# LasseWolter/laughter-detection-icsi

Measured on AMD Instinct MI355X. Metric: 1 s@16 kHz segments/sec (featurize+ResNet fwd/bwd), higher is better.
Workload: dtype f32 (64->64 and 32->32 convolutions: f16x2 split operands with per-tile power-of-two scales, f32 accumulate; error vs float64 within 1.5x of the exact-f32 kernels'); 1 GPU; BASELINE configs[2]: end-to-end featurize (HIP fbank 44 mel) + ResNetBigger resnet_base fwd/bwd + clip + Adam, random labels, dropout 0.5; global_batch=512, parallelism=dp1, overlap_wgrad=False, overlap_wgrad_small=True, bf16x3_convs=True, f16x2_convs=True, relu_bits=True, virtual_a1=True

## Files before the change

include/lad_hip.h:

```cpp
#ifndef LAD_HIP_H
#define LAD_HIP_H

#include <stdint.h>

#ifdef __cplusplus
extern "C" {
#endif

#define LAD_VERSION 100

enum lad_status {
    LAD_OK = 0,
    LAD_ERR_INVALID = -1,
    LAD_ERR_HIP = -2,
    LAD_ERR_NOMEM = -3,
    LAD_NOT_COVERED = 1
};

int lad_version(void);
const char *lad_last_error(void);

enum lad_pad_mode {
    LAD_PAD_KALDI_MIRROR = 0,
    LAD_PAD_CENTER_REFLECT = 1,
// ... 36 lines not shown
                         int32_t band, int32_t row_bytes, void *stream);


int64_t lad_act_rows(int64_t batch, int32_t H, int32_t W);

int64_t lad_conv_packed_weight_floats(int32_t cout, int32_t cin, int32_t taps, int32_t mode);
int lad_conv_pack_weights(const float *w, int32_t cout, int32_t cin, int32_t taps, int32_t mode, float *wt,
                          void *stream);
int lad_conv_pack_weights_multi(const void *descs, int32_t n_desc, void *stream);
int64_t lad_conv_num_tiles(int64_t batch, int32_t H, int32_t W);
int lad_conv_fwd(const float *in, const float *wt, const float *bias, const float *addend, float *out,
                 float *stat_partials, int64_t batch, int32_t H, int32_t W, int32_t cin, int32_t cout, int32_t taps,
                 void *stream);
int lad_conv_s2_fwd(const float *in, const float *wt, const float *bias, float *out, float *stat_partials,
                    int64_t batch, int32_t H, int32_t W, int32_t cin, int32_t cout, int32_t taps, void *stream);
int lad_bn_fold(const float *gamma, const float *beta, const float *running_mean, const float *running_var,
                const float *conv_bias, int32_t channels, float *scale, float *shift, void *stream);
int lad_conv_fwd_eval(const float *in, const float *wt, const float *scale, const float *shift, const float *addend,
                      float *out, int64_t batch, int32_t H, int32_t W, int32_t cin, int32_t cout, int32_t taps,
                      int32_t relu, void *stream);
int lad_conv_s2_fwd_eval(const float *in, const float *wt, const float *scale, const float *shift, float *out,
                         int64_t batch, int32_t H, int32_t W, int32_t cin, int32_t cout, int32_t taps, int32_t relu,
                         void *stream);
int lad_upsample2(const float *src, float *up, int64_t batch, int32_t H, int32_t W, int32_t channels, void *stream);
int lad_conv_s2_dgrad(const float *dout, const float *wt, float *dx, int64_t batch, int32_t H, int32_t W, int32_t cin,
                      int32_t cout, int32_t taps, int32_t accumulate, void *stream);
int64_t lad_conv_s2_wgrad_workspace_floats(int32_t cin, int32_t cout, int32_t taps);
int lad_conv_s2_wgrad(const float *in, const float *dout, float *workspace, float *dw, float *dbias, int64_t batch, int32_t H,
                      int32_t W, int32_t cin, int32_t cout, int32_t taps, void *stream);
int64_t lad_conv_s2_wgrad_fused_workspace_floats(int32_t cin, int32_t cout);
int lad_conv_s2_wgrad_fused(const float *in, const float *dout, const float *dout_sc, float *workspace, float *dw,
                            float *dbias, float *dw_sc, int64_t batch, int32_t H, int32_t W, int32_t cin, int32_t cout,
                            void *stream);
int lad_conv_s2_fwd_fused(const float *in, const float *wt, const float *bias, const float *wt_sc, float *out,
                          float *stat_partials, float *out_sc, float *stat_partials_sc, int64_t batch, int32_t H, int32_t W,
                          int32_t cin, int32_t cout, void *stream);
int lad_conv_s2_dgrad_fused(const float *dout, const float *wt, const float *dout_sc, const float *wt_sc, float *dx,
                            int64_t batch, int32_t H, int32_t W, int32_t cin, int32_t cout, void *stream);
int64_t lad_conv_s2b3_packed_weight_bytes(void);
int lad_conv_s2b3_pack_weights(const float *w, const float *w_sc, void *wt, void *stream);
int lad_conv_s2b3_fwd(const float *in, const void *wt, const float *bias, float *out, float *stat_partials, float *out_sc,
                      float *stat_partials_sc, int64_t batch, int32_t H, int32_t W, void *stream);
int64_t lad_conv_s2b3_dgrad_packed_weight_bytes(void);
int lad_conv_s2b3_dgrad_pack_weights(const float *w, const float *w_sc, void *wt, void *stream);
int lad_conv_s2b3_pack_weights_pair(const float *w, const float *w_sc, void *wt_fwd, void *wt_dgrad, void *stream);
int64_t lad_conv_s2b3_dgrad_partials(int64_t batch, int32_t H, int32_t W);
int lad_conv_s2b3_dgrad(const float *dout, const float *dout_sc, const void *wt, float *dx, float *stat_partials, const float *bn_x,
                        const uint64_t *bn_bits, const float *bn_coef, int64_t batch, int32_t H, int32_t W, void *stream);
int64_t lad_conv_s2_dgrad_partials(int64_t batch, int32_t H, int32_t W);
int lad_conv_s2_dgrad_fused_bnstat(const float *dout, const float *wt, const float *dout_sc, const float *wt_sc, float *dx,
                                   float *stat_partials, const float *bn_x, const uint64_t *bn_bits, const float *bn_coef,
                                   int64_t batch, int32_t H, int32_t W, int32_t cin, int32_t cout, void *stream);
int64_t lad_conv_wgrad_workspace_floats(int32_t cin, int32_t cout, int32_t taps);
int lad_conv_wgrad(const float *in, const float *dout, float *workspace, float *dw, float *dbias, int64_t batch,
                   int32_t H, int32_t W, int32_t cin, int32_t cout, int32_t taps, void *stream);

int64_t lad_conv_b3_packed_weight_bytes(void);
int lad_conv_b3_pack_weights(const float *w, int32_t mode, void *wt, void *stream);
int lad_conv_b3_fwd_f32(const float *in, const void *wt, const float *bias, const float *addend, float *out,
                        float *partials, int64_t batch, int32_t H, int32_t W, void *stream);
int lad_conv_b3_fwd_f32_gated(const float *in, const void *wt, const float *bias, const float *addend,
                              const uint64_t *addend_bits, float *out, float *partials, int64_t batch, int32_t H,
                              int32_t W, void *stream);
int lad_conv_b3_dgrad_bnstat(const float *in, const void *wt, const float *addend, const uint64_t *addend_bits,
                             float *out, float *stat_partials, const float *bn_x, const uint64_t *bn_bits,
                             const float *bn_coef, int64_t batch, int32_t H, int32_t W, void *stream);
// ... 188 lines not shown
```

laughter-detection-icsi_amd/_hip.py:

```python
import ctypes
import os

import torch

_HERE = os.path.dirname(os.path.abspath(__file__))
LIB_PATH = os.environ.get("LAD_HIP_LIB") or os.path.join(_HERE, "liblad_hip.so")

c_void_p = ctypes.c_void_p
c_int = ctypes.c_int
c_i64 = ctypes.c_int64
c_float = ctypes.c_float
c_double = ctypes.c_double
c_i32 = ctypes.c_int32
c_float_p = ctypes.POINTER(ctypes.c_float)


class LadHipError(RuntimeError):
    pass


class FbankCfg(ctypes.Structure):
    _fields_ = [("n_fft", ctypes.c_int32), ("frame_len", ctypes.c_int32), ("hop", ctypes.c_int32),
                ("n_mels", ctypes.c_int32), ("n_mfcc", ctypes.c_int32), ("pad_mode", ctypes.c_int32),
                ("log_mode", ctypes.c_int32), ("remove_dc", ctypes.c_int32), ("preemph", ctypes.c_float),
# ... 32 lines not shown
    "lad_conv_wgrad_h2": (c_int, [c_void_p] * 6 + [c_i64, c_i32, c_i32, c_i32, c_void_p]),
    "lad_conv_h2": (c_int, [c_void_p] * 11 + [c_i64, c_i32, c_i32, c_i32, c_void_p]),
    "lad_conv_wgrad_h2_bnbwd": (c_int, [c_void_p] * 11 + [c_i64, c_i32, c_i32, c_i32, c_void_p]),
    "lad_conv_wgrad_b3c_workspace_floats": (c_i64, [c_i32]),
    "lad_conv_wgrad_b3c": (c_int, [c_void_p] * 6 + [c_i64, c_i32, c_i32, c_i32, c_void_p]),
    "lad_conv_b3_fwd_f32_gated": (c_int, [c_void_p] * 7 + [c_i64, c_i32, c_i32, c_void_p]),
    "lad_conv_b3_fwd_f32_bnrelu": (c_int, [c_void_p] * 6 + [c_i64, c_i32, c_i32, c_void_p]),
    "lad_conv_wgrad_b3_bnrelu": (c_int, [c_void_p] * 6 + [c_i64, c_i32, c_i32, c_void_p]),
    "lad_wgrad_defer_begin": (c_int, []),
    "lad_wgrad_defer_flush": (c_int, [c_void_p]),
    "lad_conv_b3_dgrad_bnstat": (c_int, [c_void_p] * 9 + [c_i64, c_i32, c_i32, c_void_p]),
    "lad_conv_wgrad_b3": (c_int, [c_void_p] * 5 + [c_i64, c_i32, c_i32, c_void_p]),
    "lad_conv_s2_fwd": (c_int, [c_void_p] * 5 + [c_i64, c_i32, c_i32, c_i32, c_i32, c_i32, c_void_p]),
    "lad_bn_fold": (c_int, [c_void_p] * 5 + [c_i32, c_void_p, c_void_p, c_void_p]),
    "lad_conv_fwd_eval": (c_int, [c_void_p] * 6 + [c_i64, c_i32, c_i32, c_i32, c_i32, c_i32, c_i32, c_void_p]),
    "lad_conv_s2_fwd_eval": (c_int, [c_void_p] * 5 + [c_i64, c_i32, c_i32, c_i32, c_i32, c_i32, c_i32, c_void_p]),
    "lad_upsample2": (c_int, [c_void_p, c_void_p, c_i64, c_i32, c_i32, c_i32, c_void_p]),
    "lad_conv_s2_dgrad": (c_int, [c_void_p] * 3 + [c_i64, c_i32, c_i32, c_i32, c_i32, c_i32, c_i32, c_void_p]),
    "lad_conv_s2_wgrad_workspace_floats": (c_i64, [c_i32, c_i32, c_i32]),
    "lad_conv_s2_fwd_fused": (c_int, [c_void_p] * 8 + [c_i64, c_i32, c_i32, c_i32, c_i32, c_void_p]),
    "lad_conv_s2_dgrad_partials": (c_i64, [c_i64, c_i32, c_i32]),
    "lad_conv_s2b3_packed_weight_bytes": (c_i64, []),
    "lad_conv_s2b3_pack_weights": (c_int, [c_void_p, c_void_p, c_void_p, c_void_p]),
    "lad_conv_s2b3_fwd": (c_int, [c_void_p] * 7 + [c_i64, c_i32, c_i32, c_void_p]),
    "lad_conv_s2b3_dgrad_packed_weight_bytes": (c_i64, []),
    "lad_conv_s2b3_dgrad_pack_weights": (c_int, [c_void_p, c_void_p, c_void_p, c_void_p]),
    "lad_conv_s2b3_pack_weights_pair": (c_int, [c_void_p] * 5),
    "lad_conv_s2b3_dgrad_partials": (c_i64, [c_i64, c_i32, c_i32]),
    "lad_conv_s2b3_dgrad": (c_int, [c_void_p] * 8 + [c_i64, c_i32, c_i32, c_void_p]),
    "lad_conv_s2_dgrad_fused_bnstat": (c_int, [c_void_p] * 9 + [c_i64, c_i32, c_i32, c_i32, c_i32, c_void_p]),
    "lad_conv_s2_dgrad_fused": (c_int, [c_void_p] * 5 + [c_i64, c_i32, c_i32, c_i32, c_i32, c_void_p]),
    "lad_conv_s2_wgrad_fused_workspace_floats": (c_i64, [c_i32, c_i32]),
    "lad_conv_s2_wgrad_fused": (c_int, [c_void_p] * 7 + [c_i64, c_i32, c_i32, c_i32, c_i32, c_void_p]),
    "lad_conv_s2_wgrad": (c_int, [c_void_p] * 5 + [c_i64, c_i32, c_i32, c_i32, c_i32, c_i32, c_void_p]),
    "lad_conv_wgrad_workspace_floats": (c_i64, [c_i32, c_i32, c_i32]),
    "lad_conv_wgrad": (c_int, [c_void_p] * 5 + [c_i64, c_i32, c_i32, c_i32, c_i32, c_i32, c_void_p]),
    "lad_stem_fwd": (c_int, [c_void_p] * 4 + [c_i64, c_i32, c_i32, c_i32, c_void_p]),
    "lad_stem_fwd_eval": (c_int, [c_void_p] * 5 + [c_i64, c_i32, c_i32, c_i32, c_i64, c_i64, c_void_p]),
    "lad_stem_wgrad_workspace_floats": (c_i64, []),
    "lad_stem_wgrad": (c_int, [c_void_p] * 4 + [c_i64, c_i32, c_i32, c_i32, c_void_p]),
    "lad_stem_wgrad_bn": (c_int, [c_void_p] * 8 + [c_i64, c_i32, c_i32, c_i32, c_void_p]),
    "lad_stem_bn_bwd_groups": (c_i64, [c_i64, c_i32, c_i32]),
    "lad_stem_bn_bwd_sums": (c_int, [c_void_p] * 5 + [c_i64, c_i32, c_i32, c_i32, c_void_p]),
    "lad_bn_finalize": (c_int, [c_void_p, c_i64, c_i32, c_i64, c_void_p, c_void_p, c_void_p, c_void_p, c_float,
                                c_void_p, c_void_p]),
    "lad_stem_moments_workspace_doubles": (c_i64, []),
    "lad_stem_moments_doubles": (c_i64, []),
    "lad_stem_bn_stats": (c_int, [c_void_p] * 6 + [c_float] + [c_void_p] * 3 + [c_i64, c_i32, c_i32, c_i32, c_void_p]),
    "lad_stem_bwd_onepass_workspace_floats": (c_i64, []),
    "lad_stem_bwd_onepass": (c_int, [c_void_p] * 10 + [c_i64, c_i32, c_i32, c_i32, c_void_p]),
    "lad_bn_finalize_pair": (c_int, [c_void_p, c_void_p, c_i64, c_i32, c_i64] + [c_void_p] * 10 + [c_float, c_void_p]),
    "lad_bn_act": (c_int, [c_void_p] * 5 + [c_i64, c_i32, c_i32, c_i32, c_i32, c_void_p]),
    "lad_bn_bwd_workspace_floats": (c_i64, [c_i32]),
    "lad_bn_act_bits": (c_int, [c_void_p] * 6 + [c_i64, c_i32, c_i32, c_i32, c_void_p]),
    "lad_bn_bwd_bits": (c_int, [c_void_p] * 11 + [c_i64, c_i64, c_i32, c_i32, c_i32, c_void_p]),
    "lad_bn_bwd": (c_int, [c_void_p] * 17 + [c_i64, c_i64, c_i32, c_i32, c_i32, c_i32, c_i32, c_void_p]),
    "lad_conv_fwd_bnstat": (c_int, [c_void_p] * 8 + [c_i64, c_i32, c_i32, c_i32, c_i32, c_i32, c_void_p]),
    "lad_pool_fwd": (c_int, [c_void_p, c_void_p, c_i64, c_i32, c_i32, c_i32, c_void_p]),
    "lad_pool_bwd": (c_int, [c_void_p, c_void_p, c_i64, c_i32, c_i32, c_i32, c_void_p]),
    "lad_head_workspace_floats": (c_i64, [c_i64, c_i32]),
    "lad_head_fwd_train": (c_int, [c_void_p, c_void_p, c_i64, c_i32, c_void_p, c_void_p, c_void_p, c_float,
                                   c_void_p, c_void_p, c_void_p, c_void_p, c_void_p]),
    "lad_head_fwd_train_rng": (c_int, [c_void_p, c_void_p, c_i64, c_i32, c_void_p, c_void_p, c_float, ctypes.c_uint64, c_void_p, c_void_p, c_i32,
                                       c_void_p, c_float, c_void_p, c_void_p, c_void_p, c_void_p, c_void_p]),
    "lad_head_fwd_eval": (c_int, [c_void_p, c_void_p, c_i64, c_i32, c_void_p, c_void_p]),
    "lad_bce_metrics": (c_int, [c_void_p, c_void_p, c_i64, c_void_p, c_void_p]),
# ... 93 lines not shown
```

laughter-detection-icsi_amd/engine.py:

```python
import ctypes
import math
import struct
from typing import FrozenSet, NamedTuple, Optional, Tuple

import torch

import _hip

_VP = ctypes.c_void_p


PREDICT_CHUNK = {"fp16": 8192, "fp32": 2048}
BASE_WIDTHS = (64, 32, 16, 16)
STREAM_SUPER_MAX = 1 << 20


class _LazyLevels(dict):

    def __init__(self, make):
        super().__init__()
        self._make = make

    def __missing__(self, key):
        value = self[key] = self._make(key)
# ... 27 lines not shown
        self.wt_d = image(lib.lad_conv_packed_weight_floats(cout, cin, taps, 1), torch.float32)
        self.wt_h = image(lib.lad_f16_packed_weight_halfs(cout, cin, taps), torch.float16)
        if _b3_shape(cin, cout, taps, stride) and base_widths:
            self.wt3_f, self.wt3_d = (image(lib.lad_conv_b3c_packed_weight_bytes(cin), torch.uint8) for _ in range(2))
            self.wt2_f, self.wt2_d = (image(lib.lad_conv_h2_packed_weight_bytes(cin), torch.uint8) for _ in range(2))
        if _s2b3_shape(cin, cout, taps, stride) and base_widths:
            self.wt3_s2f = image(lib.lad_conv_s2b3_packed_weight_bytes(), torch.uint8)
            self.wt3_s2d = image(lib.lad_conv_s2b3_dgrad_packed_weight_bytes(), torch.uint8)


class _BnParams:

    def __init__(self, name, c, views, bufs, dev, conv_bias=None):
        self.name, self.c, self.conv_bias = name, c, conv_bias
        self.g, self.gg = views[name + ".weight"]
        self.b, self.gb = views[name + ".bias"]
        self.rm, self.rv = bufs[name + ".running_mean"], bufs[name + ".running_var"]
        if not (self.rm.is_cuda and self.rm.is_contiguous() and self.rm.dtype == torch.float32):
            raise _hip.LadHipError(f"{name}: running statistics must be contiguous float32 GPU tensors")
        self.fold = (torch.zeros(c, device=dev), torch.zeros(c, device=dev))


class _ConvSpec:

    def __init__(self, name, cin, cout, taps, stride, h_in, w_in, base_widths=True):
        self.name, self.cin, self.cout, self.taps, self.stride = name, cin, cout, taps, stride
        self.h_in, self.w_in = h_in, w_in
        self.h_out = (h_in + stride - 1) // stride
        self.w_out = (w_in + stride - 1) // stride
        self.b3 = _b3_shape(cin, cout, taps, stride) and w_in <= 46 and base_widths
        self.b3_full = self.b3 and cin == 64
        self.b3_wgrad = self.b3 and (cin == 64 or w_in <= 30)
        self.s2b3 = _s2b3_shape(cin, cout, taps, stride) and (w_in + 1) // 2 <= 45 and base_widths
        self.par = None

    def rows(self, B):
        return B * (self.h_in + 1) * (self.w_in + 1) + self.w_in + 2


class _BlockSpec:

    def __init__(self, name):
        self.name = name
        self.conv1 = self.bn1 = self.conv2 = self.bn2 = self.sc_conv = self.sc_bn = None


def block_geometry(stem_cout, filter_sizes, H, W, base_widths):
    blocks = []
    cin, h, w = stem_cout, H, W
    for bi, cout in enumerate(filter_sizes, start=1):
        for j in range(2):
            name = f"block{bi}.{j}"
            stride = 2 if (j == 0 and bi > 1) else 1
            b = _BlockSpec(name)
            b.conv1 = _ConvSpec(name + ".conv1", cin, cout, 9, stride, h, w, base_widths)
            h, w = b.conv1.h_out, b.conv1.w_out
            b.conv2 = _ConvSpec(name + ".conv2", cout, cout, 9, 1, h, w, base_widths)
            if stride != 1 or cin != cout:
                b.sc_conv = _ConvSpec(name + ".shortcut.0", cin, cout, 1, stride, b.conv1.h_in, b.conv1.w_in, base_widths)
            blocks.append(b)
            cin = cout
    return blocks


class _ConvChoice(NamedTuple):
    arith: str
    wgrad: str
    wgrad_bn: bool
    label_fwd: str
    label_dgrad: str


class _BlockChoice(NamedTuple):
    entry: str
    a1_virtual: bool
    bits: bool
    dgrad2_bn: Optional[str]
    dgrad1_bn: Optional[str]
    sc_wgrad_fused: bool
    conv1: _ConvChoice
    conv2: _ConvChoice
    sc: Optional[_ConvChoice]


class _TrainSchedule(NamedTuple):
    blocks: Tuple[_BlockChoice, ...]
    stem_onepass: bool
    images: FrozenSet[Tuple[str, str]]
    opts: Tuple[Tuple[str, object], ...]


_ROW_LIMIT = (1 << 31) - (1 << 20)


def train_schedule(blocks, B, opts, stem_onepass):
    o = dict(opts)

    def arith(cs):
        fits = cs.rows(B) < _ROW_LIMIT if cs.cin == 64 else cs.rows(B) * cs.cin * 4 < _ROW_LIMIT
        if not (o["bf16x3"] and cs.b3 and (cs.cin == 64 or o["bf16x3_32"]) and fits):
            return "f32"
        return "h2" if o["f16x2"] and (cs.cin == 64 or o["f16x2_32"]) else "b3"

    def conv(cs, dgrad_f32=False, label_fwd=None):
        a = arith(cs)
        wg = "f32" if a == "f32" or not cs.b3_wgrad else "h2" if a == "h2" and cs.cin == 64 else "b3c"
        f32_label = f"conv_s{cs.stride}<{cs.cin},{cs.cout},{cs.taps}>"
        return _ConvChoice(a, wg, bool(o["fuse_bn_bwd_wgrad"]) and wg == "h2",
                           label_fwd or (f32_label if a == "f32" else f"conv_{a}<{cs.cin},{cs.cout},{cs.taps}>"),
                           f"conv_s1<{cs.cout},{cs.cin},{cs.taps}>" if a == "f32" or dgrad_f32 else f"conv_{a}<{cs.cout},{cs.cin},{cs.taps}>")

    out = []
    for bi, b in enumerate(blocks):
        c1, c2, sc = b.conv1, b.conv2, b.sc_conv
        a1, a2 = arith(c1), arith(c2)
        below_bits = bi > 0 and out[bi - 1].bits
        entry = "plain"
        if c1.stride != 1 and o["fuse_s2_shortcut"]:
            entry = "s2b3" if o["bf16x3"] and o["s2_b3"] and c1.s2b3 and c1.rows(B) < _ROW_LIMIT else "s2_fused"
        bits = bool(o["relu_bits"]) and sc is None and c1.b3_full and a1 != "f32" and not o["fuse_bn_bwd"]
        dgrad2_bn = "f32" if o["fuse_bn_bwd"] else "split" if o["fuse_bn_bwd_b3"] and a2 != "f32" else None
        if c1.stride != 1:
            fused = entry == "s2b3" or (entry == "s2_fused" and c1.cin == 64 and c1.cout == 32)
            dgrad1_bn = "split" if fused and o["fuse_bn_bwd_b3"] and below_bits else None
        elif bits:
            dgrad1_bn = "split" if o["fuse_bn_bwd_b3"] and below_bits else None
        else:
            dgrad1_bn = "f32" if o["fuse_bn_bwd"] and bi > 0 and blocks[bi - 1].sc_conv is None else None
        s2_label = f"conv_{'s2b3' if entry == 's2b3' else 's2'}<{c1.cin},{c1.cout},9>" if c1.stride != 1 else None
        out.append(_BlockChoice(entry, bool(o["virtual_a1"]) and a2 != "f32" and c2.b3_wgrad, bits, dgrad2_bn, dgrad1_bn,
                                c1.stride != 1 and bool(o["fuse_s2_shortcut_wgrad"]),
                                conv(c1, dgrad1_bn == "f32", s2_label), conv(c2, dgrad2_bn == "f32"), conv(sc) if sc is not None else None))
    images = {(ch.arith if ch.arith == "h2" else "b3c", cs.name) for b, blk in zip(blocks, out)
              for cs, ch in ((b.conv1, blk.conv1), (b.conv2, blk.conv2)) if ch.arith != "f32"}
    images |= {("s2b3", b.conv1.name) for b, blk in zip(blocks, out) if blk.entry == "s2b3"}
    return _TrainSchedule(tuple(out), bool(stem_onepass), frozenset(images), tuple(o.items()))


def conv_s1_entry(arith, cin, in_coef=False, gated=False, bn=None):
    if arith == "h2" and bn != "y":
        return "lad_conv_h2"
    if arith == "b3" and in_coef and not gated and bn is None:
        return "lad_conv_b3c_fwd_f32_bnrelu"
    if arith == "b3" and gated and not in_coef and cin == 64 and bn in (None, "bits"):
        return "lad_conv_b3_dgrad_bnstat" if bn else "lad_conv_b3_fwd_f32_gated"
    if arith == "b3" and not in_coef and not gated and bn in (None, "x"):
        return "lad_conv_b3c_dgrad_bnstat" if bn else "lad_conv_b3c_fwd_f32"
    if arith == "f32" and not in_coef and not gated and bn != "bits":
        return "lad_conv_fwd_bnstat" if bn else "lad_conv_fwd"
    raise _hip.LadHipError(f"no stride-1 convolution kernel for arithmetic {arith!r} at {cin} channels with in_coef={in_coef}, "
                           f"gated={gated}, bn={bn!r}")


def conv_wgrad_entry(kind, in_coef=False, bn=False):
    if kind == "h2":
        return "lad_conv_wgrad_h2_bnbwd" if bn else "lad_conv_wgrad_h2"
    if kind == "b3c" and not bn:
        return "lad_conv_wgrad_b3c"
    if kind == "f32" and not bn and not in_coef:
        return "lad_conv_wgrad"
    raise _hip.LadHipError(f"no weight-gradient kernel for {kind!r} with in_coef={in_coef}, bn={bn}")


def _s2_shortcut_rides(b, opts):
    return bool(opts["f16_s2_shortcut_fused"]) and b.conv1.cin != 32


def _block_fits_lds(b, B, opts, hw=None):
    c = b.conv1
# ... 135 lines not shown
        self.i0, self.S, self.B_max = i0, S, B_max
        self.base, self.frames_avail = base, frames_avail
        self.cat = self.cat2 = self.stem = None


class ResNetEngine:
    KERNEL_OPTIONS =("bf16x3", "bf16x3_32", "f16x2", "f16x2_32", "relu_bits", "virtual_a1", "fuse_bn_bwd", "fuse_bn_bwd_b3", "fuse_bn_bwd_wgrad", "fuse_s2_shortcut",
                      "fuse_s2_shortcut_wgrad", "s2_b3")
    INFER_OPTIONS = ("stream_direct", "stream_level2", "stream_super", "strip_block_fused", "small_block_fused", "tail_fused", "strip2_resident",
                     "strip_stem_shared", "f16_s2_shortcut_fused")

    def __init__(self, model):
        self.model = model
        self.device = None
        self._flat_p = self._flat_g = None
        self._plans = {}
        self._step_count = 0
        self._lib = None
        self._grad_dirty = False
        self._train_forwards = 0
        self._weights_version = 0
        self.fuse_bn_bwd = False
        self.overlap_wgrad = False
        self.overlap_wgrad_small = "auto"
        self.stem_onepass = True
        self.bf16x3 = True
        self.fuse_bn_bwd_b3 = True
        self.fuse_bn_bwd_wgrad = True
        self.f16x2 = True
        self.f16x2_32 = True
        self.bf16x3_32 = True
        self.virtual_a1 = True
        self.s2_b3 = True
        self.stream_direct = True
        self.stream_level2 = True
        self.strip_block_fused = True
        self.small_block_fused = True
        self.stream_super = True
        self.tail_fused = True
        self.strip2_resident = True
        self.strip_stem_shared = True
        self._sup_cache = {}
        self._sup_plans = {}
        self._layouts = {}
        self.f16_s2_shortcut_fused = True
        self.fuse_s2_shortcut = True
        self.fuse_s2_shortcut_wgrad = True
        self.defer_wgrad_sums = True
        self._defer_on = False
        self._schedules = {}
        self.relu_bits = True
        self._side = None
        self._side_readers = {}
        self._side_pending = False
        self.debug_capture = None
        self.kernel_events = None
        self.base_widths = list(model.filter_sizes) == list(BASE_WIDTHS)
        if not self.base_widths:
            for k in self.KERNEL_OPTIONS:
                setattr(self, k, False)

    def lib(self):
        if self._lib is None:
            self._lib = _hip.lib()
        return self._lib

    def _named_params(self):
        return list(self.model.named_parameters())

    def ensure_flat(self):
        params = self._named_params()
        dev = params[0][1].device
        if dev.type != "cuda":
            raise _hip.LadHipError("ResNetBigger runs on the MI355X only: call model.set_device('cuda') first "
                                   "(the HIP path has no CPU fallback)")
        ok = self._flat_p is not None and self._flat_p.device == dev
        if ok:
            base = self._flat_p.data_ptr()
            for (name, p), off in zip(params, self._offsets):
                if p.data_ptr() != base + 4 * off or p.dtype != torch.float32:
                    ok = False
                    break
        if ok:
            return
        offs, total = [], 0
        for _, p in params:
            offs.append(total)
            total += _align4(p.numel())
        flat_p = torch.zeros(total, device=dev, dtype=torch.float32)
        flat_g = torch.zeros(total, device=dev, dtype=torch.float32)
        with torch.no_grad():
            for (name, p), off in zip(params, offs):
# ... 237 lines not shown
            _hip.check(lib.lad_conv_h2_pack_weights_multi(_hip.ptr(htab[0]), htab[1], 0, st), "lad_conv_h2_pack_weights_multi")
        self._packed = (ver, need_dgrad or have[1], want | have[2]) if fresh else (ver, need_dgrad, want)

    def _eval_prepare(self, half):
        if not half:
            self._pack_weights(need_dgrad=False)
        tag = self._state_tag()
        lib, st = self.lib(), self._st()
        if self._folded != tag:
            for bn in (self.stem_bn, *self._bns.values()):
                _hip.check(lib.lad_bn_fold(_hip.ptr(bn.g), _hip.ptr(bn.b), _hip.ptr(bn.rm), _hip.ptr(bn.rv), _hip.ptr(bn.conv_bias),
                                           bn.c, _hip.ptr(bn.fold[0]), _hip.ptr(bn.fold[1]), st), "lad_bn_fold " + bn.name)
            self._folded = tag
        if half and self._f16_packed != tag:
            for par in self._convs.values():
                _hip.check(lib.lad_f16_pack_weights(_hip.ptr(par.w), par.cout, par.cin, par.taps, _hip.ptr(par.wt_h), st),
                           "lad_f16_pack_weights " + par.name)
            self._f16_packed = tag

    def _mark(self, label):
        if self.kernel_events is None or label not in self.kernel_events:
            return None
        ev = torch.cuda.Event(enable_timing=True)
        ev.record(torch.cuda.current_stream(self.device))
        return ev

    def _mark_end(self, label, start):
        if start is not None:
            ev = torch.cuda.Event(enable_timing=True)
            ev.record(torch.cuda.current_stream(self.device))
            self.kernel_events[label].append((start, ev))

    def _schedule(self, B, H, W):
        key = (B, H, W, self.stem_onepass) + tuple(getattr(self, k) for k in self.KERNEL_OPTIONS)
        sched = self._schedules.get(key)
        if sched is None:
            sched = self._schedules[key] = train_schedule(self._blocks_for(H, W)[0], B, {k: getattr(self, k) for k in self.KERNEL_OPTIONS},
                                                          self.stem_onepass)
        return sched

    def _conv_s1(self, cs, arith, direction, x, out, B, label=None, *, in_coef=None, bias=None, addend=None, abits=None, partials=None, bn=None):
        bx, bmask, bcoef = bn if bn is not None else (None, None, None)
        fn = conv_s1_entry(arith, cs.cin, in_coef is not None, abits is not None,
                           None if bn is None else "x" if bmask is None else "bits" if bmask.dtype == torch.int64 else "y")
        P, fwd, h, w = _hip.ptr, direction == "fwd", cs.h_in, cs.w_in
        wt = P(getattr(cs.par, {"h2": "wt2_", "b3": "wt3_", "f32": "wt_"}[arith] + ("f" if fwd else "d")))
        cio = (cs.cin, cs.cout) if fwd else (cs.cout, cs.cin)
        if fn == "lad_conv_h2":
            args = (P(x), P(in_coef), wt, P(bias), P(addend), P(abits), P(out), P(partials), P(bx), P(bmask), P(bcoef), B, h, w, cs.cin)
        elif fn == "lad_conv_b3c_fwd_f32":
            args = (P(x), wt, P(bias), P(addend), P(out), P(partials), B, h, w, cs.cin)
        elif fn == "lad_conv_b3c_fwd_f32_bnrelu":
            args = (P(x), P(in_coef), wt, P(bias), P(out), P(partials), B, h, w, cs.cin)
        elif fn == "lad_conv_b3c_dgrad_bnstat":
            args = (P(x), wt, P(addend), P(out), P(partials), P(bx), P(bcoef), B, h, w, cs.cin)
        elif fn == "lad_conv_b3_fwd_f32_gated":
            args = (P(x), wt, P(bias), P(addend), P(abits), P(out), P(partials), B, h, w)
        elif fn == "lad_conv_b3_dgrad_bnstat":
            args = (P(x), wt, P(addend), P(abits), P(out), P(partials), P(bx), P(bmask), P(bcoef), B, h, w)
        elif fn == "lad_conv_fwd":
            args = (P(x), wt, P(bias), P(addend), P(out), P(partials), B, h, w, *cio, cs.taps)
        else:
            args = (P(x), wt, P(addend), P(out), P(partials), P(bx), P(bmask), P(bcoef), B, h, w, *cio, cs.taps)
        t0 = self._mark(label)
        _hip.check(getattr(self.lib(), fn)(*args, self._st()), f"{fn}({direction}) {cs.name}")
        self._mark_end(label, t0)

    def _conv_fwd(self, cs, ch, x, out, partials, B, in_coef=None):
        if cs.stride == 1:
            self._conv_s1(cs, ch.arith, "fwd", x, out, B, ch.label_fwd, in_coef=in_coef, bias=cs.par.b, partials=partials)
            return
# ... 670 lines not shown
                self._bn_bwd(p, b.bn2, dy, a["y"], a["c2"], a["coef2"], dc2, B, ho, wo, 1, mode=2, aux=aux,
                             sbn=b.sc_bn, xs=a["cs"], scoef=a["coefs"])
            xin, xcoef = (a["c1"], a["coef1"]) if ch.a1_virtual else (a["a1"], None)
            self._conv_wgrad(p, c2s, ch.conv2.wgrad, xin, dc2, B, in_coef=xcoef, bn=(dy, a["c2"], bits, a["coef2"]) if fuse2 else None)
            stat = (a["c1"], None, a["coef1"]) if ch.dgrad2_bn else None
            self._conv_s1(c2s, "f32" if ch.dgrad2_bn == "f32" else ch.conv2.arith, "dgrad", dc2, da1, B, ch.conv2.label_dgrad,
                          bn=stat, partials=p["partials"] if stat else None)
            self._bn_bwd(p, b.bn1, da1, None, a["c1"], a["coef1"], None if fuse1 else dc1, B, ho, wo, 2, mode=0, pre=stat is not None)
            if c1s.stride == 1:
                self._conv_wgrad(p, c1s, ch.conv1.wgrad, a["x"], dc1, B, bn=(da1, a["c1"], None, a["coef1"]) if fuse1 else None)
            if self.debug_capture is not None:
                self.debug_capture[b.name] = {"dy": dy.clone(), "dc2": dc2.clone(), "aux": aux.clone() if bits is None else None, "da1": da1.clone(),
                                              "dc1": dc1.clone()}
            if c1s.stride == 1:
                dx = dy
                if b.sc_conv is not None:
                    self._conv_wgrad(p, b.sc_conv, ch.sc.wgrad, a["x"], aux, B)
                    self._conv_s1(b.sc_conv, ch.sc.arith, "dgrad", aux, da1, B)
                    aux = da1
                stat = (lower["c2"], lower["ybits" if ch.dgrad1_bn == "split" else "y"], lower["coef2"]) if ch.dgrad1_bn else None
                self._conv_s1(c1s, "f32" if ch.dgrad1_bn == "f32" else ch.conv1.arith, "dgrad", dc1, dx, B, ch.conv1.label_dgrad,
                              addend=dy if ch.bits else aux, abits=bits, bn=stat, partials=p["partials"] if stat else None)
                pre2, pre2_tiles = stat is not None, 0
            else:
                dx = p["g"][(hi, wi)][0]
                sc = b.sc_conv

                def s2_wgrad(cs, dout, xin=a["x"]):
                    self._on_side(lambda sst: _hip.check(lib.lad_conv_s2_wgrad(
                        _hip.ptr(xin), _hip.ptr(dout), _hip.ptr(self._wg_ws(p, cs)), _hip.ptr(cs.par.gw), _hip.ptr(cs.par.gb), B, hi, wi, cs.cin, cs.cout,
                        cs.taps, sst), "lad_conv_s2_wgrad " + cs.name), dout, small=cs.cin <= 32)

                if ch.sc_wgrad_fused:
                    self._on_side(lambda sst, c1s=c1s, sc=sc, dc1=dc1, aux=aux, xin=a["x"]: _hip.check(lib.lad_conv_s2_wgrad_fused(
                        _hip.ptr(xin), _hip.ptr(dc1), _hip.ptr(aux), _hip.ptr(self._wg_ws(p, c1s)), _hip.ptr(c1s.par.gw), _hip.ptr(c1s.par.gb),
                        _hip.ptr(sc.par.gw), B, hi, wi, c1s.cin, c1s.cout, sst), "lad_conv_s2_wgrad_fused " + c1s.name), dc1, small=c1s.cin <= 32)
                    if dc1.data_ptr() in self._side_readers:
                        self._side_readers[aux.data_ptr()] = self._side_readers[dc1.data_ptr()]
                else:
                    s2_wgrad(c1s, dc1)
                stat = (lower["c2"], lower["ybits"], lower["coef2"]) if ch.dgrad1_bn else (None, None, None)
                n_part = 0
                if ch.entry == "s2b3":
                    n_part = int(lib.lad_conv_s2b3_dgrad_partials(B, hi, wi))
                    assert not ch.dgrad1_bn or n_part * 2 * 64 <= p["partials"].numel()
                    _hip.check(lib.lad_conv_s2b3_dgrad(_hip.ptr(dc1), _hip.ptr(aux), _hip.ptr(c1s.par.wt3_s2d), _hip.ptr(dx),
                                                       _hip.ptr(p["partials"]) if ch.dgrad1_bn else None, _hip.ptr(stat[0]), _hip.ptr(stat[1]),
                                                       _hip.ptr(stat[2]), B, hi, wi, st), "lad_conv_s2b3_dgrad " + c1s.name)
                elif ch.entry == "s2_fused" and ch.dgrad1_bn:
                    n_part = int(lib.lad_conv_s2_dgrad_partials(B, hi, wi))
                    assert n_part * 2 * 64 <= p["partials"].numel()
                    _hip.check(lib.lad_conv_s2_dgrad_fused_bnstat(_hip.ptr(dc1), _hip.ptr(c1s.par.wt_d), _hip.ptr(aux), _hip.ptr(sc.par.wt_d), _hip.ptr(dx),
                                                                  _hip.ptr(p["partials"]), _hip.ptr(stat[0]), _hip.ptr(stat[1]),
                                                                  _hip.ptr(stat[2]), B, hi, wi, c1s.cin, c1s.cout, st),
                               "lad_conv_s2_dgrad_fused_bnstat " + c1s.name)
                elif ch.entry == "s2_fused":
                    _hip.check(lib.lad_conv_s2_dgrad_fused(_hip.ptr(dc1), _hip.ptr(c1s.par.wt_d), _hip.ptr(aux), _hip.ptr(sc.par.wt_d), _hip.ptr(dx),
                                                           B, hi, wi, c1s.cin, c1s.cout, st), "lad_conv_s2_dgrad_fused " + c1s.name)
                else:
                    _hip.check(lib.lad_conv_s2_dgrad(_hip.ptr(dc1), _hip.ptr(c1s.par.wt_d), _hip.ptr(dx), B, hi, wi, c1s.cin, c1s.cout, 9, 0,
                                                     st), "lad_conv_s2_dgrad " + c1s.name)
                pre2, pre2_tiles = ch.dgrad1_bn is not None, n_part
                if not ch.sc_wgrad_fused:
                    s2_wgrad(sc, aux)
                if ch.entry == "plain":
                    _hip.check(lib.lad_conv_s2_dgrad(_hip.ptr(aux), _hip.ptr(sc.par.wt_d), _hip.ptr(dx), B, hi, wi, sc.cin, sc.cout, 1, 1, st),
                               "lad_conv_s2_dgrad " + sc.name)
            dy = dx
        if sched.stem_onepass:
# ... 134 lines not shown
```

Measured before the change: 47960 segments/s.

## Add f16x2 split-precision MFMA kernel for fused stride-2 64->32 weight gradient

Adds a new weight-gradient kernel for the stride-2 64->32 transition conv, fused with its 1x1 shortcut. It splits the input and upstream gradients into pairs of f16 values with per-tile power-of-two scales and runs f16 MFMA with transposed LDS reads. The engine selects it by default when the s2b3 entry, f16x2 and fused-shortcut options are active and the width fits one K step. The aim is to replace the previous fused wgrad path with cheaper half-precision matrix-core work. The cost is extra scaling logic, rescaling of the accumulators when the exponent drops, and a precision risk from the split operands.

Result: no change. 48410 segments/s (median of 6 runs) (+0.9%).

```diff
diff --git a/include/lad_hip.h b/include/lad_hip.h
--- a/include/lad_hip.h
+++ b/include/lad_hip.h
@@ -92,6 +92,9 @@
 int lad_conv_s2_wgrad_fused(const float *in, const float *dout, const float *dout_sc, float *workspace, float *dw,
                             float *dbias, float *dw_sc, int64_t batch, int32_t H, int32_t W, int32_t cin, int32_t cout,
                             void *stream);
+int lad_conv_s2_wgrad_fused_h2(const float *in, const float *dout, const float *dout_sc, float *workspace, float *dw,
+                               float *dbias, float *dw_sc, int64_t batch, int32_t H, int32_t W, int32_t cin, int32_t cout,
+                               void *stream);
 int lad_conv_s2_fwd_fused(const float *in, const float *wt, const float *bias, const float *wt_sc, float *out,
                           float *stat_partials, float *out_sc, float *stat_partials_sc, int64_t batch, int32_t H, int32_t W,
                           int32_t cin, int32_t cout, void *stream);
diff --git a/laughter-detection-icsi_amd/_hip.py b/laughter-detection-icsi_amd/_hip.py
--- a/laughter-detection-icsi_amd/_hip.py
+++ b/laughter-detection-icsi_amd/_hip.py
@@ -88,6 +88,7 @@
     "lad_conv_s2_dgrad_fused": (c_int, [c_void_p] * 5 + [c_i64, c_i32, c_i32, c_i32, c_i32, c_void_p]),
     "lad_conv_s2_wgrad_fused_workspace_floats": (c_i64, [c_i32, c_i32]),
     "lad_conv_s2_wgrad_fused": (c_int, [c_void_p] * 7 + [c_i64, c_i32, c_i32, c_i32, c_i32, c_void_p]),
+    "lad_conv_s2_wgrad_fused_h2": (c_int, [c_void_p] * 7 + [c_i64, c_i32, c_i32, c_i32, c_i32, c_void_p]),
     "lad_conv_s2_wgrad": (c_int, [c_void_p] * 5 + [c_i64, c_i32, c_i32, c_i32, c_i32, c_i32, c_void_p]),
     "lad_conv_wgrad_workspace_floats": (c_i64, [c_i32, c_i32, c_i32]),
     "lad_conv_wgrad": (c_int, [c_void_p] * 5 + [c_i64, c_i32, c_i32, c_i32, c_i32, c_i32, c_void_p]),
diff --git a/laughter-detection-icsi_amd/csrc/s2_h2.hip b/laughter-detection-icsi_amd/csrc/s2_h2.hip
--- /dev/null
+++ b/laughter-detection-icsi_amd/csrc/s2_h2.hip
@@ -0,0 +1,261 @@
+#include "lad_common.h"
+#include "lad_device.h"
+
+#include <algorithm>
+
+namespace {
+using namespace lad;
+
+constexpr int THREADS = 256;
+constexpr int CIN = 64, COUT = 32, TAPS = 9;
+constexpr int MAX_GROUPS = 768;
+constexpr int TK = 32;
+constexpr int IN_PITCH = 272;
+constexpr int IN_PLANE = CIN * 2;
+constexpr int DO_PITCH = COUT * 2, DO_PLANE = TK * DO_PITCH;
+constexpr int HEAD = 1;
+constexpr int CI4 = CIN / 4, CO4 = COUT / 4;
+constexpr int BPARTS = THREADS / COUT;
+
+typedef _Float16 h16x2 __attribute__((ext_vector_type(2)));
+typedef float f32x2 __attribute__((ext_vector_type(2)));
+typedef short s16x4 __attribute__((ext_vector_type(4)));
+
+__device__ __forceinline__ void split2_pair(float a, float b, unsigned &p1, unsigned &p2) {
+    const f32x2 v = {a, b};
+    const h16x2 h = __builtin_convertvector(v, h16x2);
+    p1 = __builtin_bit_cast(unsigned, h);
+    const f32x2 r = {a - (float)h.x, b - (float)h.y};
+    p2 = __builtin_bit_cast(unsigned, __builtin_convertvector(r, h16x2));
+}
+__device__ __forceinline__ int scale_exp(float amax) {
+    const int e = (int)((__builtin_bit_cast(unsigned, amax) >> 23) & 0xffu);
+    const int k = 141 - e;
+    return k > 100 ? 100 : k;
+}
+__device__ __forceinline__ float pow2f(int k) { return __builtin_bit_cast(float, (unsigned)(127 + k) << 23); }
+__device__ __forceinline__ float amax4(float4 f) { return fmaxf(fmaxf(fabsf(f.x), fabsf(f.y)), fmaxf(fabsf(f.z), fabsf(f.w))); }
+
+__device__ __forceinline__ f16x8 read_tr(unsigned addr_lo, unsigned addr_hi, int imm) {
+    typedef __attribute__((address_space(3))) s16x4 *lds_p;
+    const s16x4 lo = __builtin_amdgcn_ds_read_tr16_b64_v4i16((lds_p)(size_t)(addr_lo + imm));
+    const s16x4 hi = __builtin_amdgcn_ds_read_tr16_b64_v4i16((lds_p)(size_t)(addr_hi + imm));
+    return __builtin_bit_cast(f16x8, __builtin_shufflevector(lo, hi, 0, 1, 2, 3, 4, 5, 6, 7));
+}
+
+template <int PRE>
+__global__ __launch_bounds__(THREADS, PRE <= 9 ? 3 : 2) void wgrad_s2_h2_kernel(const float *__restrict__ in, const float *__restrict__ dout,
+                                                                const float *__restrict__ dout_sc, float *__restrict__ slabs,
+                                                                float *__restrict__ bias_slabs, float *__restrict__ slabs_sc, Geom ghi,
+                                                                Geom glo, int64_t n_tiles, int Ho) {
+    extern __shared__ __attribute__((aligned(128))) unsigned char smem_s2h[];
+    const int tid = threadIdx.x, lane = tid & 63, wave = __builtin_amdgcn_readfirstlane(tid >> 6);
+    const int span = 3 * ghi.Wp + 1;
+    const int nin = span * CI4;
+    unsigned char *in_s = smem_s2h;
+    unsigned char *do_s = in_s + span * IN_PITCH;
+    unsigned char *do2_s = do_s + 2 * DO_PLANE;
+    float *dof_s = reinterpret_cast<float *>(do2_s + 2 * DO_PLANE);
+    float *bred_s = dof_s + TK * COUT;
+    float *smx = bred_s + THREADS;
+
+    f32x4 acc[TAPS + 1][2];
+#pragma unroll
+    for (int t = 0; t <= TAPS; ++t)
+#pragma unroll
+        for (int n = 0; n < 2; ++n) acc[t][n] = f32x4{0.f, 0.f, 0.f, 0.f};
+    float bsum = 0.0f;
+    const int bco = tid % COUT, bpart = tid / COUT;
+
+    float4 pin[PRE], pdo, pdo2;
+    auto fetch = [&](int64_t tile) {
+        const int64_t b = tile / Ho;
+        const int yo = (int)(tile - b * Ho);
+        const __amdgpu_buffer_rsrc_t in_r = make_rsrc(in + ((b * ghi.Hp + 2 * yo) * (int64_t)ghi.Wp) * CIN, (int64_t)nin * 16);
+#pragma unroll
+        for (int u = 0; u < PRE; ++u) pin[u] = as_f4(buf_load16(in_r, (u * THREADS + tid) * 16));
+        const int64_t lo_row = (b * glo.Hp + yo + 1) * (int64_t)glo.Wp;
+        pdo = as_f4(buf_load16(make_rsrc(dout + lo_row * COUT, (int64_t)glo.Wp * COUT * 4), tid * 16));
+        pdo2 = as_f4(buf_load16(make_rsrc(dout_sc + lo_row * COUT, (int64_t)glo.Wp * COUT * 4), tid * 16));
+    };
+
+    const int gr = lane >> 4, w16 = lane & 15;
+    const int lrow = 4 * gr + (w16 >> 2), colb = (w16 & 3) * 8;
+    auto in_row = [&](int k) { return min(max(2 * (k - 1), 0), ghi.Wp - 2); };
+    const unsigned a_lo = lds_addr(in_s) + in_row(lrow) * IN_PITCH + wave * 32 + colb;
+    const unsigned a_hi = lds_addr(in_s) + in_row(lrow + 16) * IN_PITCH + wave * 32 + colb;
+    const unsigned b_lo = lds_addr(do_s) + lrow * DO_PITCH + colb, b_hi = b_lo + 16 * DO_PITCH;
+    const unsigned b2_lo = lds_addr(do2_s) + lrow * DO_PITCH + colb, b2_hi = b2_lo + 16 * DO_PITCH;
+    auto tap_off = [&](int tap) { return (unsigned)((tap < TAPS ? (tap / 3) * ghi.Wp + (tap % 3) : ghi.Wp + 1) * IN_PITCH); };
+    unsigned char *in_w = in_s + (tid / CI4) * IN_PITCH + (tid % CI4) * 8;
+    unsigned char *do_w = do_s + (tid / CO4) * DO_PITCH + (tid % CO4) * 8;
+
+    int e_in = 0, e_do = 0, e_sc = 0;
+    bool have = false;
+    int64_t tile = blockIdx.x;
+    if (tile < n_tiles) fetch(tile);
+    for (; tile < n_tiles; tile += gridDim.x) {
+        float m_in = 0.f;
+#pragma unroll
+        for (int u = 0; u < PRE; ++u) m_in = fmaxf(m_in, amax4(pin[u]));
+        m_in = wave_max64_dpp(m_in);
+        float m_do = wave_max64_dpp(amax4(pdo)), m_sc = wave_max64_dpp(amax4(pdo2));
+        if (lane == 0) {
+            smx[wave] = m_in;
+            smx[4 + wave] = m_do;
+            smx[8 + wave] = m_sc;
+        }
+        __syncthreads();
+        m_in = fmaxf(fmaxf(smx[0], smx[1]), fmaxf(smx[2], smx[3]));
+        m_do = fmaxf(fmaxf(smx[4], smx[5]), fmaxf(smx[6], smx[7]));
+        m_sc = fmaxf(fmaxf(smx[8], smx[9]), fmaxf(smx[10], smx[11]));
+        int d_in = 0, d_do = 0, d_sc = 0;
+        if (!have || scale_exp(m_in) < e_in) {
+            const int e_new = scale_exp(m_in) - HEAD;
+            d_in = have ? e_new - e_in : 0;
+            e_in = e_new;
+        }
+        if (!have || scale_exp(m_do) < e_do) {
+            const int e_new = scale_exp(m_do) - HEAD;
+            d_do = have ? e_new - e_do : 0;
+            e_do = e_new;
+        }
+        if (!have || scale_exp(m_sc) < e_sc) {
+            const int e_new = scale_exp(m_sc) - HEAD;
+            d_sc = have ? e_new - e_sc : 0;
+            e_sc = e_new;
+        }
+        have = true;
+        if (d_in + d_do != 0) {
+#pragma unroll
+            for (int t = 0; t < TAPS; ++t)
+#pragma unroll
+                for (int n = 0; n < 2; ++n)
+#pragma unroll
+                    for (int j = 0; j < 4; ++j) acc[t][n][j] = __builtin_ldexpf(acc[t][n][j], d_in + d_do);
+        }
+        if (d_in + d_sc != 0) {
+#pragma unroll
+            for (int n = 0; n < 2; ++n)
+#pragma unroll
+                for (int j = 0; j < 4; ++j) acc[TAPS][n][j] = __builtin_ldexpf(acc[TAPS][n][j], d_in + d_sc);
+        }
+        {
+            const float s_in = pow2f(e_in), s_do = pow2f(e_do), s_sc = pow2f(e_sc);
+            unsigned a1, a2, b1, b2;
+#pragma unroll
+            for (int u = 0; u < PRE; ++u) {
+                if (u * THREADS + tid < nin) {
+                    split2_pair(pin[u].x * s_in, pin[u].y * s_in, a1, a2);
+                    split2_pair(pin[u].z * s_in, pin[u].w * s_in, b1, b2);
+                    unsigned char *dst = in_w + u * (THREADS / CI4) * IN_PITCH;
+                    *reinterpret_cast<u32x2 *>(dst) = u32x2{a1, b1};
+                    *reinterpret_cast<u32x2 *>(dst + IN_PLANE) = u32x2{a2, b2};
+                }
+            }
+            split2_pair(pdo.x * s_do, pdo.y * s_do, a1, a2);
+            split2_pair(pdo.z * s_do, pdo.w * s_do, b1, b2);
+            *reinterpret_cast<u32x2 *>(do_w) = u32x2{a1, b1};
+            *reinterpret_cast<u32x2 *>(do_w + DO_PLANE) = u32x2{a2, b2};
+            split2_pair(pdo2.x * s_sc, pdo2.y * s_sc, a1, a2);
+            split2_pair(pdo2.z * s_sc, pdo2.w * s_sc, b1, b2);
+            *reinterpret_cast<u32x2 *>(do_w + 2 * DO_PLANE) = u32x2{a1, b1};
+            *reinterpret_cast<u32x2 *>(do_w + 3 * DO_PLANE) = u32x2{a2, b2};
+            reinterpret_cast<float4 *>(dof_s)[tid] = pdo;
+        }
+        __syncthreads();
+        if (tile + gridDim.x < n_tiles) fetch(tile + gridDim.x);
+        if (bias_slabs != nullptr) {
+            for (int r = bpart; r < glo.Wp; r += BPARTS) bsum += dof_s[r * COUT + bco];
+        }
+
+        f16x8 b[2][2];
+#pragma unroll
+        for (int n = 0; n < 2; ++n)
+#pragma unroll
+            for (int p = 0; p < 2; ++p) b[n][p] = read_tr(b_lo + n * 32, b_hi + n * 32, p * DO_PLANE);
+#pragma unroll
+        for (int tap = 0; tap <= TAPS; ++tap) {
+            const unsigned o = tap_off(tap);
+            f16x8 a[2];
+#pragma unroll
+            for (int p = 0; p < 2; ++p) a[p] = read_tr(a_lo + o, a_hi + o, p * IN_PLANE);
+            if (tap == TAPS) {
+#pragma unroll
+                for (int n = 0; n < 2; ++n)
+#pragma unroll
+                    for (int p = 0; p < 2; ++p) b[n][p] = read_tr(b2_lo + n * 32, b2_hi + n * 32, p * DO_PLANE);
+            }
+#define LAD_S2H_TERM(pa, pb) \
+    _Pragma("unroll") for (int n = 0; n < 2; ++n) acc[tap][n] = __builtin_amdgcn_mfma_f32_16x16x32_f16(a[pa], b[n][pb], acc[tap][n], 0, 0, 0);
+            LAD_S2H_TERM(0, 1)
+            LAD_S2H_TERM(1, 0)
+            LAD_S2H_TERM(0, 0)
+#undef LAD_S2H_TERM
+            __builtin_amdgcn_sched_barrier(0);
+        }
+    }
+
+    float *slab = slabs + (int64_t)blockIdx.x * (TAPS * CIN * COUT);
+    float *slab2 = slabs_sc + (int64_t)blockIdx.x * (CIN * COUT);
+#pragma unroll
+    for (int t = 0; t <= TAPS; ++t)
+#pragma unroll
+        for (int n = 0; n < 2; ++n)
+#pragma unroll
+            for (int j = 0; j < 4; ++j) {
+                const int ci = wave * 16 + 4 * gr + j, co = n * 16 + w16;
+                if (t < TAPS) slab[(t * CIN + ci) * COUT + co] = __builtin_ldexpf(acc[t][n][j], -(e_in + e_do));
+                else slab2[ci * COUT + co] = __builtin_ldexpf(acc[t][n][j], -(e_in + e_sc));
+            }
+    if (bias_slabs != nullptr) {
+        __syncthreads();
+        bred_s[bpart * COUT + bco] = bsum;
+        __syncthreads();
+        if (tid < COUT) {
+            float s = 0.0f;
+            for (int p = 0; p < BPARTS; ++p) s += bred_s[p * COUT + tid];
+            bias_slabs[(int64_t)blockIdx.x * COUT + tid] = s;
+        }
+    }
+}
+
+template <int PRE>
+int launch(const float *in, const float *dout, const float *dout_sc, float *ws, float *dw, float *dbias, float *dw_sc, int64_t batch,
+           int H, int W, hipStream_t st) {
+    const Geom ghi = make_geom(batch, H, W), glo = make_geom(batch, (H + 1) / 2, (W + 1) / 2);
+    const int Ho = (H + 1) / 2;
+    const int64_t n_tiles = batch * Ho;
+    const int groups = (int)std::max<int64_t>(1, std::min<int64_t>(MAX_GROUPS, n_tiles));
+    const size_t lds = (size_t)(3 * ghi.Wp + 1) * IN_PITCH + 4 * DO_PLANE + (TK * COUT + THREADS + 12) * sizeof(float);
+    static lad::DeviceOnce attr_set;
+    if (!attr_set) {
+        LAD_HIP_CHECK(hipFuncSetAttribute((const void *)wgrad_s2_h2_kernel<PRE>, hipFuncAttributeMaxDynamicSharedMemorySize, 96 * 1024));
+        attr_set = true;
+    }
+    float *bias_slabs = ws + (int64_t)MAX_GROUPS * TAPS * CIN * COUT;
+    float *slabs_sc = bias_slabs + (int64_t)MAX_GROUPS * COUT;
+    hipLaunchKernelGGL((wgrad_s2_h2_kernel<PRE>), dim3(groups), dim3(THREADS), lds, st, in, dout, dout_sc, ws, dbias ? bias_slabs : nullptr,
+                       slabs_sc, ghi, glo, n_tiles, Ho);
+    int rc = lad::check_launch("wgrad_s2_h2_kernel");
+    if (rc) return rc;
+    rc = lad::reduce_slabs(lad::SlabReduce{ws, dbias ? bias_slabs : nullptr, dw, dbias, groups, CIN, COUT, TAPS}, st);
+    if (rc) return rc;
+    return lad::reduce_slabs(lad::SlabReduce{slabs_sc, nullptr, dw_sc, nullptr, groups, CIN, COUT, 1}, st);
+}
+
+}
+
+extern "C" int lad_conv_s2_wgrad_fused_h2(const float *in, const float *dout, const float *dout_sc, float *workspace, float *dw,
+                                          float *dbias, float *dw_sc, int64_t batch, int32_t H, int32_t W, int32_t cin, int32_t cout,
+                                          void *stream) {
+    using namespace lad;
+    LAD_REQUIRE(in && dout && dout_sc && workspace && dw && dw_sc, "lad_conv_s2_wgrad_fused_h2: null buffer");
+    LAD_REQUIRE(batch >= 1 && H >= 1 && W >= 1, "lad_conv_s2_wgrad_fused_h2: bad geometry");
+    LAD_REQUIRE(cin == CIN && cout == COUT, "lad_conv_s2_wgrad_fused_h2: the 64 -> 32 transition only (got cin=%d, cout=%d)", cin, cout);
+    LAD_REQUIRE((W + 1) / 2 + 1 <= TK, "lad_conv_s2_wgrad_fused_h2: %d padded low-resolution columns exceed one K step of %d (W = %d)",
+                (W + 1) / 2 + 1, TK, W);
+    if ((3 * (W + 1) + 1) * CI4 <= 9 * THREADS)
+        return launch<9>(in, dout, dout_sc, workspace, dw, dbias, dw_sc, batch, H, W, (hipStream_t)stream);
+    return launch<12>(in, dout, dout_sc, workspace, dw, dbias, dw_sc, batch, H, W, (hipStream_t)stream);
+}
diff --git a/laughter-detection-icsi_amd/engine.py b/laughter-detection-icsi_amd/engine.py
--- a/laughter-detection-icsi_amd/engine.py
+++ b/laughter-detection-icsi_amd/engine.py
@@ -83,6 +83,7 @@
         self.b3_full = self.b3 and cin == 64
         self.b3_wgrad = self.b3 and (cin == 64 or w_in <= 30)
         self.s2b3 = _s2b3_shape(cin, cout, taps, stride) and (w_in + 1) // 2 <= 45 and base_widths
+        self.s2h2_wgrad = self.s2b3 and (w_in + 1) // 2 + 1 <= 32
         self.par = None
 
     def rows(self, B):
@@ -132,6 +133,7 @@
     conv1: _ConvChoice
     conv2: _ConvChoice
     sc: Optional[_ConvChoice]
+    sc_wgrad_h2: bool = False
 
 
 class _TrainSchedule(NamedTuple):
@@ -139,12 +141,13 @@
     stem_onepass: bool
     images: FrozenSet[Tuple[str, str]]
     opts: Tuple[Tuple[str, object], ...]
+    s2_h2: bool = True
 
 
 _ROW_LIMIT = (1 << 31) - (1 << 20)
 
 
-def train_schedule(blocks, B, opts, stem_onepass):
+def train_schedule(blocks, B, opts, stem_onepass, s2_h2=True):
     o = dict(opts)
 
     def arith(cs):
@@ -181,11 +184,12 @@
         s2_label = f"conv_{'s2b3' if entry == 's2b3' else 's2'}<{c1.cin},{c1.cout},9>" if c1.stride != 1 else None
         out.append(_BlockChoice(entry, bool(o["virtual_a1"]) and a2 != "f32" and c2.b3_wgrad, bits, dgrad2_bn, dgrad1_bn,
                                 c1.stride != 1 and bool(o["fuse_s2_shortcut_wgrad"]),
-                                conv(c1, dgrad1_bn == "f32", s2_label), conv(c2, dgrad2_bn == "f32"), conv(sc) if sc is not None else None))
+                                conv(c1, dgrad1_bn == "f32", s2_label), conv(c2, dgrad2_bn == "f32"), conv(sc) if sc is not None else None,
+                                bool(s2_h2) and entry == "s2b3" and bool(o["f16x2"]) and bool(o["fuse_s2_shortcut_wgrad"]) and c1.s2h2_wgrad))
     images = {(ch.arith if ch.arith == "h2" else "b3c", cs.name) for b, blk in zip(blocks, out)
               for cs, ch in ((b.conv1, blk.conv1), (b.conv2, blk.conv2)) if ch.arith != "f32"}
     images |= {("s2b3", b.conv1.name) for b, blk in zip(blocks, out) if blk.entry == "s2b3"}
-    return _TrainSchedule(tuple(out), bool(stem_onepass), frozenset(images), tuple(o.items()))
+    return _TrainSchedule(tuple(out), bool(stem_onepass), frozenset(images), tuple(o.items()), bool(s2_h2))
 
 
 def conv_s1_entry(arith, cin, in_coef=False, gated=False, bn=None):
@@ -387,6 +391,7 @@
         self.bf16x3_32 = True
         self.virtual_a1 = True
         self.s2_b3 = True
+        self.s2_h2 = True
         self.stream_direct = True
         self.stream_level2 = True
         self.strip_block_fused = True
@@ -412,7 +417,7 @@
         self.kernel_events = None
         self.base_widths = list(model.filter_sizes) == list(BASE_WIDTHS)
         if not self.base_widths:
-            for k in self.KERNEL_OPTIONS:
+            for k in self.KERNEL_OPTIONS + ("s2_h2",):
                 setattr(self, k, False)
 
     def lib(self):
@@ -716,11 +721,11 @@
             self.kernel_events[label].append((start, ev))
 
     def _schedule(self, B, H, W):
-        key = (B, H, W, self.stem_onepass) + tuple(getattr(self, k) for k in self.KERNEL_OPTIONS)
+        key = (B, H, W, self.stem_onepass, self.s2_h2) + tuple(getattr(self, k) for k in self.KERNEL_OPTIONS)
         sched = self._schedules.get(key)
         if sched is None:
             sched = self._schedules[key] = train_schedule(self._blocks_for(H, W)[0], B, {k: getattr(self, k) for k in self.KERNEL_OPTIONS},
-                                                          self.stem_onepass)
+                                                          self.stem_onepass, self.s2_h2)
         return sched
 
     def _conv_s1(self, cs, arith, direction, x, out, B, label=None, *, in_coef=None, bias=None, addend=None, abits=None, partials=None, bn=None):
@@ -1457,9 +1462,10 @@
                         cs.taps, sst), "lad_conv_s2_wgrad " + cs.name), dout, small=cs.cin <= 32)
 
                 if ch.sc_wgrad_fused:
-                    self._on_side(lambda sst, c1s=c1s, sc=sc, dc1=dc1, aux=aux, xin=a["x"]: _hip.check(lib.lad_conv_s2_wgrad_fused(
+                    fn = "lad_conv_s2_wgrad_fused_h2" if ch.sc_wgrad_h2 else "lad_conv_s2_wgrad_fused"
+                    self._on_side(lambda sst, c1s=c1s, sc=sc, dc1=dc1, aux=aux, xin=a["x"], fn=fn: _hip.check(getattr(lib, fn)(
                         _hip.ptr(xin), _hip.ptr(dc1), _hip.ptr(aux), _hip.ptr(self._wg_ws(p, c1s)), _hip.ptr(c1s.par.gw), _hip.ptr(c1s.par.gb),
-                        _hip.ptr(sc.par.gw), B, hi, wi, c1s.cin, c1s.cout, sst), "lad_conv_s2_wgrad_fused " + c1s.name), dc1, small=c1s.cin <= 32)
+                        _hip.ptr(sc.par.gw), B, hi, wi, c1s.cin, c1s.cout, sst), fn + " " + c1s.name), dc1, small=c1s.cin <= 32)
                     if dc1.data_ptr() in self._side_readers:
                         self._side_readers[aux.data_ptr()] = self._side_readers[dc1.data_ptr()]
                 else:
```
